# viniciusmenesessouza/VAE-GAN-based-model-for-image-generation-and-denoising

Hardware: AMD Instinct MI355X
Metric: images/sec/GPU VAE-GAN train step (higher is better)
Workload: dtype bf16; 1 GPU; CelebA-shaped 64x64 VAE-GAN full train step (E+G+5xD fwd, all bwd, 4 Adam), batch 128/GPU, global batch 128; img_size=64, per_gpu_batch=128, global_batch=128, parallelism=dp1, elide_dead_grads=False, hip_graph=True, hip_graph_segments=1

## Files before the change

vae-gan-based-model-for-image-generation-and-denoising_amd/csrc/bn_act.hip:

```cpp
#include "common.hpp"

namespace {

struct RedPlan { int nparts, rows_per_part, ncolblk; };

inline RedPlan plan_reduce(int64_t rows, int C) {
    const int cols = C / 4;
    const int ncol = cols < 256 ? cols : 256;
    const int rpp = 256 / ncol;
    const int64_t passes = (rows + rpp - 1) / rpp;
    int64_t np = passes / 8;
    if (np < 1) np = 1;
    if (np > 1024) np = 1024;
    int64_t rows_per_part = ((passes + np - 1) / np) * rpp;
    RedPlan p;
    p.nparts = (int)((rows + rows_per_part - 1) / rows_per_part);
    p.rows_per_part = (int)rows_per_part;
    p.ncolblk = (cols + 255) / 256;
    return p;
}

template <int DT, int MODE>
__global__ __launch_bounds__(256) void col_reduce_kernel(const void* __restrict__ x, const void* __restrict__ dy,
                                                         const float* __restrict__ scale,
// ... 169 lines not shown

__global__ __launch_bounds__(FIN_CH * FIN_PL) void bn_bwd_finalize_grouped_kernel(
    const float* __restrict__ partial, int nparts, int groups, int C, double count, const float* __restrict__ gamma,
    const float* __restrict__ coeffs, float* __restrict__ dgamma, float* __restrict__ dbeta, int accumulate,
    float* __restrict__ coef) {
    for (int g = 0; g < groups; ++g) {
        double s1, s2;
        int c;
        const bool lead = slab_sums(partial + (int64_t)g * nparts * 2 * C, nparts, C, s1, s2, c);
        if (lead) {
            const float fs1 = (float)s1, fs2 = (float)s2;
            const bool acc = accumulate || g > 0;
            if (dgamma) dgamma[c] = acc ? dgamma[c] + fs2 : fs2;
            if (dbeta) dbeta[c] = acc ? dbeta[c] + fs1 : fs1;
            const float a = (gamma ? gamma[c] : 1.f) * coeffs[(int64_t)g * 4 * C + C + c];
            float* cf = coef + (int64_t)g * 3 * C;
            cf[c] = a;
            cf[C + c] = (float)((double)a * s2 / count);
            cf[2 * C + c] = (float)((double)a * s1 / count);
        }
        __syncthreads();
    }
}

__global__ __launch_bounds__(FIN_CH * FIN_PL) void slab_sums_kernel(const float* __restrict__ slabs, int nparts, int C,
                                                                    double* __restrict__ sums) {
    double s1, s2;
    int c;
    if (!slab_sums(slabs, nparts, C, s1, s2, c)) return;
    sums[c] = s1;
    sums[C + c] = s2;
}

__global__ void bn_finalize_sums_kernel(const double* __restrict__ sums, int C, double count,
                                        const float* __restrict__ gamma, const float* __restrict__ beta,
                                        float* __restrict__ rmean, float* __restrict__ rvar, float momentum, float eps,
                                        float* __restrict__ mean, float* __restrict__ invstd,
                                        float* __restrict__ scale, float* __restrict__ shift) {
    const int c = blockIdx.x * blockDim.x + threadIdx.x;
    if (c >= C) return;
    const double mu = sums[c] / count;
    double var = sums[C + c] / count - mu * mu;
    if (var < 0.0) var = 0.0;
    const float is = (float)(1.0 / sqrt(var + (double)eps));
    const float muf = (float)mu;
    mean[c] = muf;
    invstd[c] = is;
    const float g = gamma ? gamma[c] : 1.f, b = beta ? beta[c] : 0.f;
    const float sc = g * is;
    scale[c] = sc;
    shift[c] = b - muf * sc;
    if (rmean) {
        const double unbiased = count > 1.0 ? var * (count / (count - 1.0)) : var;
        rmean[c] = (1.f - momentum) * rmean[c] + momentum * muf;
        rvar[c] = (1.f - momentum) * rvar[c] + momentum * (float)unbiased;
    }
}

__global__ void bn_bwd_finalize_sums_kernel(const double* __restrict__ gsums, const double* __restrict__ lsums, int C,
                                            double count, const float* __restrict__ gamma,
                                            const float* __restrict__ invstd, float* __restrict__ dgamma,
                                            float* __restrict__ dbeta, int accumulate, float* __restrict__ coef) {
    const int c = blockIdx.x * blockDim.x + threadIdx.x;
    if (c >= C) return;
    const float l1 = (float)lsums[c], l2 = (float)lsums[C + c];
    if (dgamma) dgamma[c] = accumulate ? dgamma[c] + l2 : l2;
    if (dbeta) dbeta[c] = accumulate ? dbeta[c] + l1 : l1;
    const float a = (gamma ? gamma[c] : 1.f) * invstd[c];
    coef[c] = a;
    coef[C + c] = (float)((double)a * gsums[C + c] / count);
    coef[2 * C + c] = (float)((double)a * gsums[c] / count);
}

__global__ void bn_eval_kernel(const float* gamma, const float* beta, const float* rmean, const float* rvar,
                               float eps, int C, float* scale, float* shift) {
    const int c = blockIdx.x * blockDim.x + threadIdx.x;
    if (c >= C) return;
    const float is = 1.f / sqrtf(rvar[c] + eps);
    const float sc = (gamma ? gamma[c] : 1.f) * is;
    scale[c] = sc;
    shift[c] = (beta ? beta[c] : 0.f) - rmean[c] * sc;
}

template <int DT>
__global__ __launch_bounds__(256) void bn_act_fwd_kernel(const void* __restrict__ x, void* __restrict__ y,
                                                         const float* __restrict__ scale,
                                                         const float* __restrict__ shift, int64_t nvec, int cols,
                                                         int act, float slope, int64_t nvec_per_group,
                                                         int64_t gstride, uint32_t* __restrict__ y8) {
    auto one = [&](int64_t i, float4 v) {
        const int c4 = (int)(i % cols) * 4;
        if (scale) {
            const int64_t go = (i / nvec_per_group) * gstride;
            const float4 sc = *reinterpret_cast<const float4*>(scale + go + c4);
            const float4 sh = *reinterpret_cast<const float4*>(shift + go + c4);
            v.x = sc.x * v.x + sh.x; v.y = sc.y * v.y + sh.y; v.z = sc.z * v.z + sh.z; v.w = sc.w * v.w + sh.w;
        }
        v.x = act_fwd(v.x, act, slope); v.y = act_fwd(v.y, act, slope);
        v.z = act_fwd(v.z, act, slope); v.w = act_fwd(v.w, act, slope);
        store4<DT>(y, i * 4, v);
        if (y8) {
            if constexpr (DT == VG_BF16) {
                v.x = ElemT<VG_BF16>::to_f32(ElemT<VG_BF16>::from_f32(v.x));
                v.y = ElemT<VG_BF16>::to_f32(ElemT<VG_BF16>::from_f32(v.y));
                v.z = ElemT<VG_BF16>::to_f32(ElemT<VG_BF16>::from_f32(v.z));
                v.w = ElemT<VG_BF16>::to_f32(ElemT<VG_BF16>::from_f32(v.w));
            }
            int w = __builtin_amdgcn_cvt_pk_fp8_f32(v.x, v.y, 0, false);
            w = __builtin_amdgcn_cvt_pk_fp8_f32(v.z, v.w, w, true);
            y8[i] = (uint32_t)w;
        }
    };
    const int64_t stride = (int64_t)gridDim.x * blockDim.x;
    int64_t i = (int64_t)blockIdx.x * blockDim.x + threadIdx.x;
    for (; i + 3 * stride < nvec; i += 4 * stride) {
        float4 v[4];
#pragma unroll
        for (int u = 0; u < 4; ++u) v[u] = load4<DT>(x, (i + u * stride) * 4);
#pragma unroll
        for (int u = 0; u < 4; ++u) one(i + u * stride, v[u]);
    }
    for (; i < nvec; i += stride) one(i, load4<DT>(x, i * 4));
}

__global__ __launch_bounds__(FIN_CH * FIN_PL) void bn_bwd_finalize_kernel(
    const float* __restrict__ partial, int nparts, int C, double count, const float* __restrict__ gamma,
    const float* __restrict__ invstd, float* __restrict__ dgamma, float* __restrict__ dbeta, int accumulate,
    float* __restrict__ coef) {
    double s1, s2;
    int c;
    if (!slab_sums(partial, nparts, C, s1, s2, c)) return;
    const float fs1 = (float)s1, fs2 = (float)s2;
    if (dgamma) dgamma[c] = accumulate ? dgamma[c] + fs2 : fs2;
    if (dbeta) dbeta[c] = accumulate ? dbeta[c] + fs1 : fs1;
    const float a = (gamma ? gamma[c] : 1.f) * invstd[c];
    coef[c] = a;
    coef[C + c] = (float)((double)a * s2 / count);
    coef[2 * C + c] = (float)((double)a * s1 / count);
}

template <int DT>
__global__ __launch_bounds__(256) void bn_act_bwd_apply_kernel(const void* __restrict__ x, const void* __restrict__ dy,
                                                               void* __restrict__ dx,
                                                               const float* __restrict__ scale,
                                                               const float* __restrict__ shift,
                                                               const float* __restrict__ mean,
                                                               const float* __restrict__ invstd,
                                                               const float* __restrict__ coef, int64_t nvec, int cols,
                                                               int C, int act, float slope, int64_t nvec_per_group,
                                                               int64_t gstride, int64_t cstride) {
    auto one = [&](int64_t i, const float4& v, const float4& g) {
        const int c4 = (int)(i % cols) * 4;
        const int64_t grp = i / nvec_per_group;
        const int64_t go = grp * gstride;
        const float* cf = coef + grp * cstride;
        const float4 sc = *reinterpret_cast<const float4*>(scale + go + c4);
        const float4 sh = *reinterpret_cast<const float4*>(shift + go + c4);
        const float4 mu = *reinterpret_cast<const float4*>(mean + go + c4);
        const float4 is = *reinterpret_cast<const float4*>(invstd + go + c4);
        const float4 ca = *reinterpret_cast<const float4*>(cf + c4);
        const float4 cbv = *reinterpret_cast<const float4*>(cf + C + c4);
        const float4 cc = *reinterpret_cast<const float4*>(cf + 2 * C + c4);
        float4 o;
        o.x = ca.x * act_bwd(sc.x * v.x + sh.x, g.x, act, slope) - cbv.x * ((v.x - mu.x) * is.x) - cc.x;
        o.y = ca.y * act_bwd(sc.y * v.y + sh.y, g.y, act, slope) - cbv.y * ((v.y - mu.y) * is.y) - cc.y;
        o.z = ca.z * act_bwd(sc.z * v.z + sh.z, g.z, act, slope) - cbv.z * ((v.z - mu.z) * is.z) - cc.z;
        o.w = ca.w * act_bwd(sc.w * v.w + sh.w, g.w, act, slope) - cbv.w * ((v.w - mu.w) * is.w) - cc.w;
        store4<DT>(dx, i * 4, o);
    };
    const int64_t stride = (int64_t)gridDim.x * blockDim.x;
    int64_t i = (int64_t)blockIdx.x * blockDim.x + threadIdx.x;
    for (; i + 3 * stride < nvec; i += 4 * stride) {
        float4 v[4], g[4];
#pragma unroll
        for (int u = 0; u < 4; ++u) { v[u] = load4<DT>(x, (i + u * stride) * 4); g[u] = load4<DT>(dy, (i + u * stride) * 4); }
#pragma unroll
        for (int u = 0; u < 4; ++u) one(i + u * stride, v[u], g[u]);
    }
    for (; i < nvec; i += stride) one(i, load4<DT>(x, i * 4), load4<DT>(dy, i * 4));
}

constexpr int FF_CH = 64, FF_PL = 16, FF_TH = FF_CH * FF_PL, FF_MAXPARTS = 200;
constexpr int64_t FF_MAXBYTES = 9ll << 20;

__device__ __forceinline__ void ff_slice_stats(const float* __restrict__ slabs, int nparts, int C, int c0, double count,
                                               double (*red)[FF_CH][2], double& mu_out, double& var_out) {
    const int ch = threadIdx.x & (FF_CH - 1), pl = threadIdx.x / FF_CH;
    double a = 0.0, b = 0.0;
    for (int p = pl; p < nparts; p += FF_PL) {
        a += (double)slabs[((int64_t)p * 2 + 0) * C + c0 + ch];
        b += (double)slabs[((int64_t)p * 2 + 1) * C + c0 + ch];
    }
    red[pl][ch][0] = a;
    red[pl][ch][1] = b;
    __syncthreads();
    double s1 = 0.0, s2 = 0.0;
#pragma unroll
    for (int k = 0; k < FF_PL; ++k) { s1 += red[k][ch][0]; s2 += red[k][ch][1]; }
    const double mu = s1 / count;
    double var = s2 / count - mu * mu;
    if (var < 0.0) var = 0.0;
    mu_out = mu;
    var_out = var;
    __syncthreads();
}

__global__ __launch_bounds__(FF_TH) void bn_fin_act_fwd_kernel(
    const uint16_t* __restrict__ x, uint16_t* __restrict__ y, const float* __restrict__ stats, int nparts, int groups,
    int C, double count, const float* __restrict__ gamma, const float* __restrict__ beta, float* __restrict__ rmean,
    float* __restrict__ rvar, float momentum, float eps, float* __restrict__ coeffs, int64_t rows_per_group,
    int rows_per_block, int act, float slope) {
    __shared__ double red[FF_PL][FF_CH][2];
    __shared__ float s_sc[FF_CH], s_sh[FF_CH];
    const int tid = threadIdx.x, ch = tid & (FF_CH - 1);
    const int c0 = blockIdx.y * FF_CH, grp = blockIdx.z;
    const bool lead = tid < FF_CH && c0 + ch < C;
    const float gm = (lead && gamma) ? gamma[c0 + ch] : 1.f, bt = (lead && beta) ? beta[c0 + ch] : 0.f;
    if (blockIdx.x == 0 && grp == 0) {
        float rm = (lead && rmean) ? rmean[c0 + ch] : 0.f, rv = (lead && rmean) ? rvar[c0 + ch] : 0.f;
        for (int g = 0; g < groups; ++g) {
            double mu, var;
            ff_slice_stats(stats + (int64_t)g * nparts * 2 * C, nparts, C, c0, count, red, mu, var);
            if (lead) {
                const float is = (float)(1.0 / sqrt(var + (double)eps));
                const float muf = (float)mu, sc = gm * is, sh = bt - muf * sc;
                float* co = coeffs + (int64_t)g * 4 * C + c0 + ch;
                co[0] = muf; co[C] = is; co[2 * C] = sc; co[3 * C] = sh;
                if (g == 0) { s_sc[ch] = sc; s_sh[ch] = sh; }
                if (rmean) {
                    const double unbiased = count > 1.0 ? var * (count / (count - 1.0)) : var;
                    rm = (1.f - momentum) * rm + momentum * muf;
                    rv = (1.f - momentum) * rv + momentum * (float)unbiased;
                }
            }
        }
        if (lead && rmean) { rmean[c0 + ch] = rm; rvar[c0 + ch] = rv; }
    } else {
        double mu, var;
        ff_slice_stats(stats + (int64_t)grp * nparts * 2 * C, nparts, C, c0, count, red, mu, var);
        if (lead) {
            const float is = (float)(1.0 / sqrt(var + (double)eps));
            const float muf = (float)mu, sc = gm * is;
            s_sc[ch] = sc;
            s_sh[ch] = bt - muf * sc;
        }
    }
    __syncthreads();
    const int u8 = (tid & 7) * 8, rl = tid >> 3;
    float sc[8], sh[8];
#pragma unroll
    for (int k = 0; k < 8; ++k) { sc[k] = s_sc[u8 + k]; sh[k] = s_sh[u8 + k]; }
    const int64_t r0 = (int64_t)blockIdx.x * rows_per_block;
    const int64_t r1 = r0 + rows_per_block < rows_per_group ? r0 + rows_per_block : rows_per_group;
    const int64_t base = (int64_t)grp * rows_per_group;
    if (c0 + u8 < C) {
        for (int64_t r = r0 + rl; r < r1; r += FF_TH / 8) {
            const int64_t off = (base + r) * C + c0 + u8;
            const u32x4 v = *reinterpret_cast<const u32x4*>(x + off);
            u32x4 o;
#pragma unroll
            for (int k2 = 0; k2 < 4; ++k2) {
                const float lo = act_fwd(sc[2 * k2] * __uint_as_float(v[k2] << 16) + sh[2 * k2], act, slope);
// ... 217 lines not shown
    return VG_LAUNCH_RC();
}

extern "C" int vg_bn_backward_finalize_sums(const double* global_sums, const double* local_sums, int C, int64_t count,
                                            const float* gamma, const float* invstd, float* dgamma, float* dbeta,
                                            int accumulate, float* coef, void* stream) {
    VG_CHECK_ARG(global_sums && local_sums && C > 0 && count > 0 && invstd && coef, VG_EINVAL);
    vg_launch_timed(4, bn_bwd_finalize_sums_kernel, dim3((C + 255) / 256), dim3(256), 0, vg_stream(stream),
                       global_sums, local_sums, C, (double)count, gamma, invstd, dgamma, dbeta, accumulate, coef);
    return VG_LAUNCH_RC();
}

extern "C" int vg_bn_eval_coeffs(const float* gamma, const float* beta, const float* running_mean,
                                 const float* running_var, float eps, int C, float* scale, float* shift,
                                 void* stream) {
    VG_CHECK_ARG(running_mean && running_var && scale && shift && C > 0, VG_EINVAL);
    vg_launch_timed(4, bn_eval_kernel, dim3((C + 63) / 64), dim3(64), 0, vg_stream(stream), gamma, beta, running_mean,
                       running_var, eps, C, scale, shift);
    return VG_LAUNCH_RC();
}

extern "C" int vg_bn_finalize_act_forward_supported(int nparts_per_group, int groups, int C, int64_t rows, int dtype) {
    return bn_fin_fwd_ok(nparts_per_group, groups, C, rows, dtype) ? 1 : 0;
}

extern "C" int vg_bn_finalize_act_forward(const void* x, void* y, const float* stats, int nparts_per_group, int groups,
                                          int C, int64_t rows, const float* gamma, const float* beta,
                                          float* running_mean, float* running_var, float momentum, float eps,
                                          float* coeffs, int act, float slope, int dtype, void* stream) {
    VG_CHECK_ARG(x && y && stats && coeffs && rows > 0 && C > 0, VG_EINVAL);
    VG_CHECK_ARG((running_mean == nullptr) == (running_var == nullptr), VG_EINVAL);
    VG_CHECK_ARG(vg_aligned16(x) && vg_aligned16(y), VG_EALIGN);
    if (!bn_fin_fwd_ok(nparts_per_group, groups, C, rows, dtype)) return VG_ENOSUP;
    const int64_t rpg = rows / groups;
    const int slices = C / FF_CH;
    int64_t want = 512 / (slices * groups);
    if (want < 1) want = 1;
    int64_t rpb = (rpg + want - 1) / want;
    rpb = (rpb + 127) / 128 * 128;
    const int rb = (int)((rpg + rpb - 1) / rpb);
    vg_launch_timed(4, bn_fin_act_fwd_kernel, dim3(rb, slices, groups), dim3(FF_TH), 0, vg_stream(stream),
                       reinterpret_cast<const uint16_t*>(x), reinterpret_cast<uint16_t*>(y), stats, nparts_per_group, groups,
                       C, (double)rpg, gamma, beta, running_mean, running_var, momentum, eps, coeffs, rpg, (int)rpb, act,
                       slope);
    return VG_LAUNCH_RC();
}

extern "C" int vg_bn_backward_finalize_apply(const void* x, const void* dy, void* dx, const float* partial,
                                             int nparts_per_group, int groups, int C, int64_t rows, const float* gamma,
                                             const float* coeffs, float* dgamma, float* dbeta, int accumulate, int act,
                                             float slope, int dtype, void* stream) {
    VG_CHECK_ARG(x && dy && dx && partial && coeffs && rows > 0 && C > 0, VG_EINVAL);
    VG_CHECK_ARG(vg_aligned16(x) && vg_aligned16(dy) && vg_aligned16(dx), VG_EALIGN);
    if (!bn_fin_fwd_ok(nparts_per_group, groups, C, rows, dtype)) return VG_ENOSUP;
    const int64_t rpg = rows / groups;
    const int slices = C / FF_CH;
    int64_t want = 512 / (slices * groups);
    if (want < 1) want = 1;
    int64_t rpb = (rpg + want - 1) / want;
    rpb = (rpb + 127) / 128 * 128;
    const int rb = (int)((rpg + rpb - 1) / rpb);
    vg_launch_timed(4, bn_bwd_fin_apply_kernel, dim3(rb, slices, groups), dim3(FF_TH), 0, vg_stream(stream),
                       reinterpret_cast<const uint16_t*>(x), reinterpret_cast<const uint16_t*>(dy),
                       reinterpret_cast<uint16_t*>(dx), partial, nparts_per_group, groups, C, (double)rpg, gamma, coeffs,
                       dgamma, dbeta, accumulate, rpg, (int)rpb, act, slope);
    return VG_LAUNCH_RC();
}

extern "C" int vg_bn_act_forward_fp8(const void* x, void* y, void* y8, const float* scale, const float* shift, int64_t rows,
                                     int C, int act, float slope, int groups, int64_t gstride, int dtype, void* stream);

extern "C" int vg_bn_act_forward(const void* x, void* y, const float* scale, const float* shift, int64_t rows, int C,
                                 int act, float slope, int groups, int64_t gstride, int dtype, void* stream) {
    return vg_bn_act_forward_fp8(x, y, nullptr, scale, shift, rows, C, act, slope, groups, gstride, dtype, stream);
}

extern "C" int vg_bn_act_forward_fp8(const void* x, void* y, void* y8, const float* scale, const float* shift, int64_t rows,
                                     int C, int act, float slope, int groups, int64_t gstride, int dtype, void* stream) {
    int rc = check_rows_c(x, rows, C, dtype);
    if (rc) return rc;
    VG_CHECK_ARG(y != nullptr && (scale == nullptr) == (shift == nullptr), VG_EINVAL);
    VG_CHECK_ARG(groups >= 1 && rows % groups == 0, VG_EINVAL);
    VG_CHECK_ARG(y8 == nullptr || (dtype == VG_BF16 && (reinterpret_cast<uintptr_t>(y8) & 3u) == 0), VG_EINVAL);
    const int64_t nvec = rows * C / 4;
    const int64_t nvg = nvec / groups;
    if (dtype == VG_F32)
        vg_launch_timed(4, bn_act_fwd_kernel<VG_F32>, dim3(ew_blocks(nvec)), dim3(256), 0, vg_stream(stream), x, y,
                           scale, shift, nvec, C / 4, act, slope, nvg, gstride, (uint32_t*)nullptr);
    else
        vg_launch_timed(4, bn_act_fwd_kernel<VG_BF16>, dim3(ew_blocks(nvec)), dim3(256), 0, vg_stream(stream), x, y,
                           scale, shift, nvec, C / 4, act, slope, nvg, gstride, reinterpret_cast<uint32_t*>(y8));
    return VG_LAUNCH_RC();
}

extern "C" int vg_channel_stats(const void* x, int64_t rows, int C, float* stats, int stats_capacity,
                                int* nparts_out, int dtype, void* stream) {
    int rc = check_rows_c(x, rows, C, dtype);
    if (rc) return rc;
    return launch_reduce<0>(x, nullptr, nullptr, nullptr, nullptr, nullptr, rows, C, 0, 0.f, stats, stats_capacity,
                            nparts_out, dtype, vg_stream(stream));
}

extern "C" int vg_bn_act_backward_reduce(const void* x, const void* dy, const float* scale, const float* shift,
                                         const float* mean, const float* invstd, int64_t rows, int C, int act,
                                         float slope, float* partial, int partial_capacity, int* nparts_out,
                                         int groups, int64_t gstride, int dtype, void* stream) {
    int rc = check_rows_c(x, rows, C, dtype);
    if (rc) return rc;
    VG_CHECK_ARG(dy && scale && shift && mean && invstd, VG_EINVAL);
    return launch_reduce<1>(x, dy, scale, shift, mean, invstd, rows, C, act, slope, partial, partial_capacity,
                            nparts_out, dtype, vg_stream(stream), groups, gstride);
}

extern "C" int vg_bn_backward_finalize(const float* partial, int nparts, int C, int64_t count, const float* gamma,
                                       const float* invstd, float* dgamma, float* dbeta, int accumulate, float* coef,
                                       void* stream) {
    VG_CHECK_ARG(partial && nparts > 0 && C > 0 && count > 0 && invstd && coef, VG_EINVAL);
    vg_launch_timed(4, bn_bwd_finalize_kernel, dim3((C + FIN_CH - 1) / FIN_CH), dim3(FIN_CH * FIN_PL), 0, vg_stream(stream), partial, nparts, C,
                       (double)count, gamma, invstd, dgamma, dbeta, accumulate, coef);
    return VG_LAUNCH_RC();
}

extern "C" int vg_bn_act_backward_apply(const void* x, const void* dy, void* dx, const float* scale,
                                        const float* shift, const float* mean, const float* invstd, const float* coef,
                                        int64_t rows, int C, int act, float slope, int groups, int64_t gstride,
                                        int64_t cstride, int dtype, void* stream) {
    int rc = check_rows_c(x, rows, C, dtype);
    if (rc) return rc;
    VG_CHECK_ARG(dy && dx && scale && shift && mean && invstd && coef, VG_EINVAL);
    VG_CHECK_ARG(groups >= 1 && rows % groups == 0, VG_EINVAL);
    const int64_t nvec = rows * C / 4;
    const int64_t nvg = nvec / groups;
    if (dtype == VG_F32)
        vg_launch_timed(4, bn_act_bwd_apply_kernel<VG_F32>, dim3(ew_blocks(nvec)), dim3(256), 0, vg_stream(stream), x,
                           dy, dx, scale, shift, mean, invstd, coef, nvec, C / 4, C, act, slope, nvg, gstride, cstride);
    else
        vg_launch_timed(4, bn_act_bwd_apply_kernel<VG_BF16>, dim3(ew_blocks(nvec)), dim3(256), 0, vg_stream(stream), x,
                           dy, dx, scale, shift, mean, invstd, coef, nvec, C / 4, C, act, slope, nvg, gstride, cstride);
    return VG_LAUNCH_RC();
}

extern "C" int vg_act_backward(const void* x, const void* dy, void* dx, int64_t n, int act, float slope, int dtype,
                               void* stream) {
    VG_CHECK_ARG(x && dy && dx && n > 0 && n % 4 == 0, VG_EINVAL);
    VG_CHECK_ARG(dtype == VG_F32 || dtype == VG_BF16, VG_ENOSUP);
    const int64_t nvec = n / 4;
    if (dtype == VG_F32)
        vg_launch_timed(4, act_bwd_kernel<VG_F32>, dim3(ew_blocks(nvec)), dim3(256), 0, vg_stream(stream), x, dy, dx,
                           nvec, act, slope);
    else
        vg_launch_timed(4, act_bwd_kernel<VG_BF16>, dim3(ew_blocks(nvec)), dim3(256), 0, vg_stream(stream), x, dy, dx,
                           nvec, act, slope);
    return VG_LAUNCH_RC();
}

extern "C" int vg_bias_grad(const void* dy, int64_t rows, int C, int NC, float* dbias, int accumulate, float* ws,
                            int ws_capacity, int dtype, void* stream) {
    int rc = check_rows_c(dy, rows, C, dtype);
    if (rc) return rc;
    VG_CHECK_ARG(dbias && ws && NC > 0 && NC <= C, VG_EINVAL);
    int nparts = 0;
    rc = launch_reduce<0>(dy, nullptr, nullptr, nullptr, nullptr, nullptr, rows, C, 0, 0.f, ws, ws_capacity, &nparts,
                          dtype, vg_stream(stream));
    if (rc) return rc;
    vg_launch_timed(4, bias_finalize_kernel, dim3((C + FIN_CH - 1) / FIN_CH), dim3(FIN_CH * FIN_PL), 0, vg_stream(stream), ws, nparts, C, NC,
                       dbias, accumulate);
    return VG_LAUNCH_RC();
}
```

vae-gan-based-model-for-image-generation-and-denoising_amd/csrc/common.hpp:

```cpp
#pragma once
#include <hip/hip_runtime.h>
#include <stdint.h>
#include "vaegan_hip.h"

typedef __attribute__((ext_vector_type(4))) float f32x4;
typedef __attribute__((ext_vector_type(8))) __bf16 bf16x8;
typedef __attribute__((ext_vector_type(4))) uint32_t u32x4;

#define VG_CHECK_ARG(cond, code) do { if (!(cond)) return (code); } while (0)

#include <atomic>
std::atomic<uint64_t>& vg_launch_counter();
#undef hipLaunchKernelGGL
#define hipLaunchKernelGGL(kernelName, numBlocks, numThreads, memPerBlock, streamId, ...)                       \
    do {                                                                                                        \
        vg_launch_counter().fetch_add(1, std::memory_order_relaxed);                                            \
        kernelName<<<(numBlocks), (numThreads), (memPerBlock), (streamId)>>>(__VA_ARGS__);                      \
    } while (0)
#define VG_LAUNCH_RC() ((int)hipGetLastError())

static inline hipStream_t vg_stream(void* s) { return reinterpret_cast<hipStream_t>(s); }
static inline bool vg_aligned16(const void* p) { return (reinterpret_cast<uintptr_t>(p) & 15u) == 0; }

template <int DT> struct ElemT;
// ... 50 lines not shown
}
template <int DT> __device__ __forceinline__ float load1(const void* base, int64_t idx) {
    return ElemT<DT>::to_f32(reinterpret_cast<const typename ElemT<DT>::type*>(base)[idx]);
}
template <int DT> __device__ __forceinline__ void store1(void* base, int64_t idx, float v) {
    reinterpret_cast<typename ElemT<DT>::type*>(base)[idx] = ElemT<DT>::from_f32(v);
}

__device__ __forceinline__ float act_fwd(float z, int act, float slope) {
    if (act == VG_ACT_RELU) return z > 0.f ? z : 0.f;
    if (act == VG_ACT_LRELU) return z > 0.f ? z : z * slope;
    return z;
}
__device__ __forceinline__ float act_bwd(float z, float g, int act, float slope) {
    if (act == VG_ACT_RELU) return z > 0.f ? g : 0.f;
    if (act == VG_ACT_LRELU) return z > 0.f ? g : g * slope;
    return g;
}

__device__ __forceinline__ float wave_sum(float v) {
#pragma unroll
    for (int o = 32; o > 0; o >>= 1) v += __shfl_xor(v, o);
    return v;
}
__device__ __forceinline__ double wave_sum_d(double v) {
#pragma unroll
    for (int o = 32; o > 0; o >>= 1) v += __shfl_xor(v, o);
    return v;
}

#include <hip/hip_ext.h>
#include <mutex>
#include <vector>
struct VgTiming {
    bool on = false;
    std::mutex mu;
    std::vector<hipEvent_t> pool;
    std::vector<std::pair<hipEvent_t, hipEvent_t>> rec[5];
};
VgTiming& vg_timing();

template <typename K, typename... Args>
inline void vg_launch_timed(int family, K kernel, dim3 grid, dim3 block, size_t shm, hipStream_t s, Args... args) {
    VgTiming& t = vg_timing();
    if (!t.on) {
        hipLaunchKernelGGL(kernel, grid, block, shm, s, args...);
        return;
    }
    hipEvent_t e0, e1;
    {
        std::lock_guard<std::mutex> g(t.mu);
        auto get = [&]() { hipEvent_t e; if (t.pool.empty()) { (void)hipEventCreate(&e); } else { e = t.pool.back(); t.pool.pop_back(); } return e; };
        e0 = get(); e1 = get();
        t.rec[family].push_back({e0, e1});
    }
    vg_launch_counter().fetch_add(1, std::memory_order_relaxed);
    hipExtLaunchKernelGGL(kernel, grid, block, shm, s, e0, e1, 0, args...);
}

struct VgSwitches {
    int gg_dma;
    int tile_min_wgs;
    int gg_patch;
    int gg_patch64;
    int gg_patch32;
    int gg_phase4;
    int gg_phase4_min;
    int gg_patch_nr3;
    int patch256_min;
    int patch256x64_min;
    int splitk_max_tiles;
    int splitk_general;
    int splitk_bigk;
    int splitk_wgs;
    int gg_nmajor;
    int edge;
    int wg_reduce_t;
    int wg_target;
    int wg_spec;
    int wg_dma;
    int wg_xcd;
    int bn_fused_fwd;
    int bn_onepass;
};
const VgSwitches& vg_sw();
```

vae-gan-based-model-for-image-generation-and-denoising_amd/csrc/pointwise.hip:

```cpp
#include "common.hpp"
#include "noise.hpp"

namespace {

__global__ __launch_bounds__(256) void cast_fp8_kernel(const u32x4* __restrict__ x, uint2* __restrict__ y, int64_t nvec,
                                                       float scale) {
    for (int64_t i = (int64_t)blockIdx.x * blockDim.x + threadIdx.x; i < nvec; i += (int64_t)gridDim.x * blockDim.x) {
        const u32x4 v = x[i];
        float f[8];
#pragma unroll
        for (int k = 0; k < 4; ++k) {
            f[2 * k] = __uint_as_float(v[k] << 16) * scale;
            f[2 * k + 1] = __uint_as_float(v[k] & 0xffff0000u) * scale;
        }
        uint2 o;
        int w = 0;
        w = __builtin_amdgcn_cvt_pk_fp8_f32(f[0], f[1], w, false);
        w = __builtin_amdgcn_cvt_pk_fp8_f32(f[2], f[3], w, true);
        o.x = (uint32_t)w;
        w = 0;
        w = __builtin_amdgcn_cvt_pk_fp8_f32(f[4], f[5], w, false);
        w = __builtin_amdgcn_cvt_pk_fp8_f32(f[6], f[7], w, true);
        o.y = (uint32_t)w;
        y[i] = o;
// ... 856 lines not shown
    VG_CHECK_ARG(B * groups <= HB_MAXROWS, VG_ENOSUP);
    DISPATCH_DT(head_bwd_kernel, dim3((K + 63) / 64), dim3(1024), vg_stream(stream), p, x, w, dx, dw, dlogit, B, groups,
                target0, target1, gscale, loss, accumulate_loss, accumulate_dw, K, C, HW);
    return VG_LAUNCH_RC();
}

extern "C" int vg_mean_forward_backward(const float* p, float sign, int B, float gscale, float* loss, int accumulate,
                                        float* dp, void* stream) {
    VG_CHECK_ARG(p && loss && B > 0, VG_EINVAL);
    hipLaunchKernelGGL(mean_loss_kernel, dim3(1), dim3(256), 0, vg_stream(stream), p, sign, B, gscale, loss, accumulate, dp);
    return VG_LAUNCH_RC();
}

extern "C" int vg_clamp(float* p, int64_t n, float lo, float hi, void* stream) {
    VG_CHECK_ARG(p && n > 0 && lo <= hi, VG_EINVAL);
    hipLaunchKernelGGL(clamp_kernel, dim3(blocks_for(n)), dim3(256), 0, vg_stream(stream), p, n, lo, hi);
    return VG_LAUNCH_RC();
}

extern "C" int vg_mse_forward_backward(const float* a, const float* b, int64_t n, float gscale, float* loss, float* d_a,
                                       float* ws, int ws_capacity, void* stream) {
    VG_CHECK_ARG(a && b && loss && ws && n > 0 && ws_capacity >= 1, VG_EINVAL);
    VG_CHECK_ARG(vg_aligned16(a) && vg_aligned16(b) && (d_a == nullptr || vg_aligned16(d_a)), VG_EALIGN);
    int blocks = blocks_for(n / 4, 1024);
    if (blocks > ws_capacity) blocks = ws_capacity;
    const float gcoef = (float)((double)gscale * 2.0 / (double)n);
    hipLaunchKernelGGL(mse_partial_kernel, dim3(blocks), dim3(256), 0, vg_stream(stream), a, b, n, gcoef, d_a, ws);
    int rc = VG_LAUNCH_RC();
    if (rc) return rc;
    hipLaunchKernelGGL(mse_final_kernel, dim3(1), dim3(64), 0, vg_stream(stream), ws, blocks, (double)n, loss);
    return VG_LAUNCH_RC();
}

extern "C" int vg_ssim(const float* a, const float* b, int B, int C, int H, int W, float* out, float* ws,
                       int ws_capacity, void* stream) {
    VG_CHECK_ARG(a && b && out && ws && B > 0 && C > 0 && H > 10 && W > 10 && ws_capacity >= 1, VG_EINVAL);
    const int64_t total = (int64_t)B * C * (H - 10) * (W - 10);
    int blocks = blocks_for(total, 1024);
    if (blocks > ws_capacity) blocks = ws_capacity;
    hipLaunchKernelGGL(ssim_kernel, dim3(blocks), dim3(256), 0, vg_stream(stream), a, b, B * C, H, W, ws);
    int rc = VG_LAUNCH_RC();
    if (rc) return rc;
    hipLaunchKernelGGL(mse_final_kernel, dim3(1), dim3(64), 0, vg_stream(stream), ws, blocks, (double)total, out);
    return VG_LAUNCH_RC();
}

extern "C" int vg_axpy(const float* a, const float* b, float alpha, float* out, int64_t n, void* stream) {
    VG_CHECK_ARG(a && b && out && n > 0, VG_EINVAL);
    hipLaunchKernelGGL(axpy_kernel, dim3(blocks_for(n)), dim3(256), 0, vg_stream(stream), a, b, alpha, out, n);
    return VG_LAUNCH_RC();
}

#include <cstdlib>
namespace {
VgSwitches g_sw;
int env_int(const char* name, int dflt) {
    const char* e = getenv(name);
    return e ? atoi(e) : dflt;
}
void read_switches() {
    g_sw.gg_dma = env_int("VG_GG_DMA", 1);
    g_sw.tile_min_wgs = env_int("VG_TILE_MIN_WGS", 512);
    g_sw.gg_patch = env_int("VG_GG_PATCH", 1);
    g_sw.gg_patch64 = env_int("VG_GG_PATCH64", 1);
    g_sw.gg_patch32 = env_int("VG_GG_PATCH32", 1);
    g_sw.gg_phase4 = env_int("VG_GG_PHASE4", 1);
    g_sw.gg_phase4_min = env_int("VG_GG_PHASE4_MIN", 512);
    g_sw.gg_patch_nr3 = env_int("VG_GG_PATCH_NR3", 1);
    g_sw.patch256_min = env_int("VG_PATCH256_MIN", 256);
    g_sw.patch256x64_min = env_int("VG_PATCH256X64_MIN", 512);
    g_sw.splitk_max_tiles = env_int("VG_SPLITK_MAX_TILES", 128);
    g_sw.splitk_wgs = env_int("VG_SPLITK_WGS", 1024);
    g_sw.splitk_bigk = env_int("VG_SPLITK_BIGK", 1);
    g_sw.splitk_general = env_int("VG_SPLITK_GENERAL", 0);
    g_sw.gg_nmajor = env_int("VG_GG_NMAJOR", 1);
    g_sw.edge = env_int("VG_EDGE", 1);
    g_sw.wg_reduce_t = env_int("VG_WG_REDUCE_T", 1);
    g_sw.wg_target = env_int("VG_WG_TARGET", 512);
    g_sw.wg_spec = env_int("VG_WG_SPEC", 3);
    g_sw.wg_dma = env_int("VG_WG_DMA", 1);
    g_sw.wg_xcd = env_int("VG_WG_XCD", 1);
    g_sw.bn_fused_fwd = env_int("VG_BN_FUSED_FWD", 1);
    g_sw.bn_onepass = env_int("VG_BN_ONEPASS", 0);
}
struct SwitchInit { SwitchInit() { read_switches(); } } g_switch_init;
}
const VgSwitches& vg_sw() { return g_sw; }
extern "C" int vg_reload_switches(void) {
    read_switches();
    return 0;
}

VgTiming& vg_timing() {
    static VgTiming t;
    return t;
}

std::atomic<uint64_t>& vg_launch_counter() {
    static std::atomic<uint64_t> n{0};
    return n;
}

extern "C" uint64_t vg_launch_count(void) { return vg_launch_counter().load(std::memory_order_relaxed); }

extern "C" int vg_timing_enable(int on) {
    VgTiming& t = vg_timing();
    std::lock_guard<std::mutex> g(t.mu);
    t.on = on != 0;
    return 0;
}

extern "C" int vg_timing_collect(int family, double* total_ms, int* launches) {
    VG_CHECK_ARG(family >= 0 && family < 5 && total_ms && launches, VG_EINVAL);
    VgTiming& t = vg_timing();
    std::lock_guard<std::mutex> g(t.mu);
    double sum = 0.0;
    for (auto& pr : t.rec[family]) {
        (void)hipEventSynchronize(pr.second);
        float ms = 0.f;
        if (hipEventElapsedTime(&ms, pr.first, pr.second) == hipSuccess) sum += ms;
        t.pool.push_back(pr.first);
        t.pool.push_back(pr.second);
    }
    *total_ms = sum;
    *launches = (int)t.rec[family].size();
    t.rec[family].clear();
    return 0;
}

extern "C" int vg_abi_version(void) { return VG_ABI_VERSION; }
extern "C" const char* vg_build_info(void) { return "vaegan_hip gfx950: gather-GEMM f32(16x16x4)/bf16(16x16x32) MFMA"; }
```

Baseline: 47980 images/sec.

## Restructure BN-activation apply kernels into row-blocked column-stationary streaming with wide vectors

```diff
diff --git a/vae-gan-based-model-for-image-generation-and-denoising_amd/csrc/bn_act.hip b/vae-gan-based-model-for-image-generation-and-denoising_amd/csrc/bn_act.hip
--- a/vae-gan-based-model-for-image-generation-and-denoising_amd/csrc/bn_act.hip
+++ b/vae-gan-based-model-for-image-generation-and-denoising_amd/csrc/bn_act.hip
@@ -275,45 +275,154 @@
     shift[c] = (beta ? beta[c] : 0.f) - rmean[c] * sc;
 }
 
-template <int DT>
+constexpr int EW_UNROLL = 4;
+constexpr int EW_FWD_WGS = 1024, EW_BWD_WGS = 768;
+inline bool stream_wide(int dtype, int64_t rows, int C) {
+    return dtype == VG_BF16 && C % 8 == 0 && rows * C * 2 >= (int64_t)vg_sw().bn_wide_min;
+}
+
+struct StreamPlan { int rows_per_block, blocks_per_group, ncolblk; };
+
+inline StreamPlan plan_stream(int64_t rows_per_group, int cols, int groups, int max_wgs) {
+    const int ncol = cols < 256 ? cols : 256;
+    const int rpp = 256 / ncol;
+    StreamPlan p;
+    p.ncolblk = (cols + 255) / 256;
+    const int64_t passes = (rows_per_group + rpp - 1) / rpp;
+    int64_t cap = max_wgs / ((int64_t)groups * p.ncolblk);
+    if (cap < 1) cap = 1;
+    const int64_t blocks = passes < cap ? passes : cap;
+    const int64_t rpb = (passes + blocks - 1) / blocks * rpp;
+    p.rows_per_block = (int)rpb;
+    p.blocks_per_group = (int)((rows_per_group + rpb - 1) / rpb);
+    return p;
+}
+
+template <int DT, int VW> struct RawVec { typedef __attribute__((ext_vector_type(VW / 2))) uint32_t type; };
+template <int VW> struct RawVec<VG_F32, VW> { typedef float4 type; };
+template <int DT, int VW>
+__device__ __forceinline__ typename RawVec<DT, VW>::type loadv(const void* base, int64_t idx) {
+    typedef typename RawVec<DT, VW>::type W;
+    return *reinterpret_cast<const W*>(reinterpret_cast<const typename ElemT<DT>::type*>(base) + idx);
+}
+template <int DT, int VW>
+__device__ __forceinline__ void unpackv(const typename RawVec<DT, VW>::type& r, float (&v)[VW]) {
+    if constexpr (DT == VG_F32) {
+        static_assert(VW == 4, "f32: one 16-byte vector");
+        v[0] = r.x; v[1] = r.y; v[2] = r.z; v[3] = r.w;
+    } else {
+#pragma unroll
+        for (int k = 0; k < VW / 2; ++k) {
+            v[2 * k] = __uint_as_float(r[k] << 16);
+            v[2 * k + 1] = __uint_as_float(r[k] & 0xffff0000u);
+        }
+    }
+}
+template <int DT, int VW> __device__ __forceinline__ void storev(void* base, int64_t idx, const float (&v)[VW]) {
+    typename RawVec<DT, VW>::type r;
+    if constexpr (DT == VG_F32) {
+        r = float4{v[0], v[1], v[2], v[3]};
+    } else {
+#pragma unroll
+        for (int k = 0; k < VW / 2; ++k)
+            r[k] = (uint32_t)ElemT<VG_BF16>::from_f32(v[2 * k]) | ((uint32_t)ElemT<VG_BF16>::from_f32(v[2 * k + 1]) << 16);
+    }
+    *reinterpret_cast<typename RawVec<DT, VW>::type*>(reinterpret_cast<typename ElemT<DT>::type*>(base) + idx) = r;
+}
+template <int V> struct IntC { static constexpr int value = V; };
+
+template <int VW> __device__ __forceinline__ void load_coef(const float* __restrict__ p, float (&c)[VW]) {
+#pragma unroll
+    for (int k = 0; k < VW; k += 4) {
+        const float4 r = *reinterpret_cast<const float4*>(p + k);
+        c[k] = r.x; c[k + 1] = r.y; c[k + 2] = r.z; c[k + 3] = r.w;
+    }
+}
+
+template <int VW>
+__device__ __forceinline__ void stream_range(int64_t rows, int C, int64_t rows_per_group, int rows_per_block, int& c,
+                                             int& rpp, int64_t& r0, int64_t& r1) {
+    const int cols = C / VW;
+    const int cb = blockIdx.y * 256;
+    const int ncol = min(256, cols - cb);
+    rpp = 256 / ncol;
+    const int tr = threadIdx.x / ncol, tc = threadIdx.x - tr * ncol;
+    c = (cb + tc) * VW;
+    const int64_t gbase = (int64_t)blockIdx.z * rows_per_group;
+    const int64_t b0 = gbase + (int64_t)blockIdx.x * rows_per_block;
+    r1 = min(min(rows, gbase + rows_per_group), b0 + (int64_t)rows_per_block);
+    r0 = tr < rpp ? b0 + tr : r1;
+}
+
+template <int DT, int VW>
 __global__ __launch_bounds__(256) void bn_act_fwd_kernel(const void* __restrict__ x, void* __restrict__ y,
                                                          const float* __restrict__ scale,
-                                                         const float* __restrict__ shift, int64_t nvec, int cols,
-                                                         int act, float slope, int64_t nvec_per_group,
-                                                         int64_t gstride, uint32_t* __restrict__ y8) {
-    auto one = [&](int64_t i, float4 v) {
-        const int c4 = (int)(i % cols) * 4;
-        if (scale) {
-            const int64_t go = (i / nvec_per_group) * gstride;
-            const float4 sc = *reinterpret_cast<const float4*>(scale + go + c4);
-            const float4 sh = *reinterpret_cast<const float4*>(shift + go + c4);
-            v.x = sc.x * v.x + sh.x; v.y = sc.y * v.y + sh.y; v.z = sc.z * v.z + sh.z; v.w = sc.w * v.w + sh.w;
-        }
-        v.x = act_fwd(v.x, act, slope); v.y = act_fwd(v.y, act, slope);
-        v.z = act_fwd(v.z, act, slope); v.w = act_fwd(v.w, act, slope);
-        store4<DT>(y, i * 4, v);
-        if (y8) {
-            if constexpr (DT == VG_BF16) {
-                v.x = ElemT<VG_BF16>::to_f32(ElemT<VG_BF16>::from_f32(v.x));
-                v.y = ElemT<VG_BF16>::to_f32(ElemT<VG_BF16>::from_f32(v.y));
-                v.z = ElemT<VG_BF16>::to_f32(ElemT<VG_BF16>::from_f32(v.z));
-                v.w = ElemT<VG_BF16>::to_f32(ElemT<VG_BF16>::from_f32(v.w));
-            }
-            int w = __builtin_amdgcn_cvt_pk_fp8_f32(v.x, v.y, 0, false);
-            w = __builtin_amdgcn_cvt_pk_fp8_f32(v.z, v.w, w, true);
-            y8[i] = (uint32_t)w;
+                                                         const float* __restrict__ shift, int64_t rows, int C, int act,
+                                                         float slope, int64_t rows_per_group, int rows_per_block,
+                                                         int64_t gstride, uint8_t* __restrict__ y8) {
+    int c, rpp;
+    int64_t r, r1;
+    stream_range<VW>(rows, C, rows_per_group, rows_per_block, c, rpp, r, r1);
+    typedef typename RawVec<DT, VW>::type Raw;
+    const int64_t step = (int64_t)rpp * C;
+    int64_t off = r * C + c;
+    float sc[VW], sh[VW];
+    if (scale) {
+        load_coef<VW>(scale + (int64_t)blockIdx.z * gstride + c, sc);
+        load_coef<VW>(shift + (int64_t)blockIdx.z * gstride + c, sh);
+    }
+    auto run = [&](auto act_c, auto affine_c) {
+        constexpr int ACT = decltype(act_c)::value;
+        constexpr bool AFFINE = decltype(affine_c)::value;
+        auto one = [&](int64_t o, const Raw& raw) {
+            float f[VW];
+            unpackv<DT, VW>(raw, f);
+            if (AFFINE) {
+#pragma unroll
+                for (int k = 0; k < VW; ++k) f[k] = __builtin_fmaf(sc[k], f[k], sh[k]);
+            }
+#pragma unroll
+            for (int k = 0; k < VW; ++k) f[k] = act_fwd(f[k], ACT, slope);
+            storev<DT, VW>(y, o, f);
+            if (y8) {
+                if constexpr (DT == VG_BF16) {
+#pragma unroll
+                    for (int k = 0; k < VW; ++k) f[k] = ElemT<VG_BF16>::to_f32(ElemT<VG_BF16>::from_f32(f[k]));
+                }
+                typedef __attribute__((ext_vector_type(VW / 4))) uint32_t W8;
+                W8 w8;
+#pragma unroll
+                for (int k = 0; k < VW / 4; ++k) {
+                    int w = __builtin_amdgcn_cvt_pk_fp8_f32(f[4 * k], f[4 * k + 1], 0, false);
+                    w = __builtin_amdgcn_cvt_pk_fp8_f32(f[4 * k + 2], f[4 * k + 3], w, true);
+                    w8[k] = (uint32_t)w;
+                }
+                *reinterpret_cast<W8*>(y8 + o) = w8;
+            }
+        };
+        for (; r + (EW_UNROLL - 1) * rpp < r1; r += EW_UNROLL * rpp, off += EW_UNROLL * step) {
+            Raw v[EW_UNROLL];
+#pragma unroll
+            for (int u = 0; u < EW_UNROLL; ++u) v[u] = loadv<DT, VW>(x, off + u * step);
+#pragma unroll
+            for (int u = 0; u < EW_UNROLL; ++u) one(off + u * step, v[u]);
+        }
+        if (r < r1) {
+            Raw v[EW_UNROLL - 1];
+#pragma unroll
+            for (int u = 0; u < EW_UNROLL - 1; ++u)
+                if (r + u * rpp < r1) v[u] = loadv<DT, VW>(x, off + u * step);
+#pragma unroll
+            for (int u = 0; u < EW_UNROLL - 1; ++u)
+                if (r + u * rpp < r1) one(off + u * step, v[u]);
         }
     };
-    const int64_t stride = (int64_t)gridDim.x * blockDim.x;
-    int64_t i = (int64_t)blockIdx.x * blockDim.x + threadIdx.x;
-    for (; i + 3 * stride < nvec; i += 4 * stride) {
-        float4 v[4];
-#pragma unroll
-        for (int u = 0; u < 4; ++u) v[u] = load4<DT>(x, (i + u * stride) * 4);
-#pragma unroll
-        for (int u = 0; u < 4; ++u) one(i + u * stride, v[u]);
-    }
-    for (; i < nvec; i += stride) one(i, load4<DT>(x, i * 4));
+    auto with_act = [&](auto affine_c) {
+        if (act == VG_ACT_RELU) run(IntC<VG_ACT_RELU>{}, affine_c);
+        else if (act == VG_ACT_LRELU) run(IntC<VG_ACT_LRELU>{}, affine_c);
+        else run(IntC<VG_ACT_NONE>{}, affine_c);
+    };
+    if (scale) with_act(IntC<1>{}); else with_act(IntC<0>{});
 }
 
 __global__ __launch_bounds__(FIN_CH * FIN_PL) void bn_bwd_finalize_kernel(
@@ -332,45 +441,66 @@
     coef[2 * C + c] = (float)((double)a * s1 / count);
 }
 
-template <int DT>
+template <int DT, int VW>
 __global__ __launch_bounds__(256) void bn_act_bwd_apply_kernel(const void* __restrict__ x, const void* __restrict__ dy,
                                                                void* __restrict__ dx,
                                                                const float* __restrict__ scale,
                                                                const float* __restrict__ shift,
                                                                const float* __restrict__ mean,
                                                                const float* __restrict__ invstd,
-                                                               const float* __restrict__ coef, int64_t nvec, int cols,
-                                                               int C, int act, float slope, int64_t nvec_per_group,
-                                                               int64_t gstride, int64_t cstride) {
-    auto one = [&](int64_t i, const float4& v, const float4& g) {
-        const int c4 = (int)(i % cols) * 4;
-        const int64_t grp = i / nvec_per_group;
-        const int64_t go = grp * gstride;
-        const float* cf = coef + grp * cstride;
-        const float4 sc = *reinterpret_cast<const float4*>(scale + go + c4);
-        const float4 sh = *reinterpret_cast<const float4*>(shift + go + c4);
-        const float4 mu = *reinterpret_cast<const float4*>(mean + go + c4);
-        const float4 is = *reinterpret_cast<const float4*>(invstd + go + c4);
-        const float4 ca = *reinterpret_cast<const float4*>(cf + c4);
-        const float4 cbv = *reinterpret_cast<const float4*>(cf + C + c4);
-        const float4 cc = *reinterpret_cast<const float4*>(cf + 2 * C + c4);
-        float4 o;
-        o.x = ca.x * act_bwd(sc.x * v.x + sh.x, g.x, act, slope) - cbv.x * ((v.x - mu.x) * is.x) - cc.x;
-        o.y = ca.y * act_bwd(sc.y * v.y + sh.y, g.y, act, slope) - cbv.y * ((v.y - mu.y) * is.y) - cc.y;
-        o.z = ca.z * act_bwd(sc.z * v.z + sh.z, g.z, act, slope) - cbv.z * ((v.z - mu.z) * is.z) - cc.z;
-        o.w = ca.w * act_bwd(sc.w * v.w + sh.w, g.w, act, slope) - cbv.w * ((v.w - mu.w) * is.w) - cc.w;
-        store4<DT>(dx, i * 4, o);
+                                                               const float* __restrict__ coef, int64_t rows, int C,
+                                                               int act, float slope, int64_t rows_per_group,
+                                                               int rows_per_block, int64_t gstride, int64_t cstride) {
+    int c, rpp;
+    int64_t r, r1;
+    stream_range<VW>(rows, C, rows_per_group, rows_per_block, c, rpp, r, r1);
+    typedef typename RawVec<DT, VW>::type Raw;
+    const int64_t step = (int64_t)rpp * C;
+    int64_t off = r * C + c;
+    float sc[VW], sh[VW], mu[VW], is[VW], ca[VW], cbv[VW], cc[VW];
+    const int64_t go = (int64_t)blockIdx.z * gstride + c;
+    const float* cf = coef + (int64_t)blockIdx.z * cstride + c;
+    load_coef<VW>(scale + go, sc);
+    load_coef<VW>(shift + go, sh);
+    load_coef<VW>(mean + go, mu);
+    load_coef<VW>(invstd + go, is);
+    load_coef<VW>(cf, ca);
+    load_coef<VW>(cf + C, cbv);
+    load_coef<VW>(cf + 2 * C, cc);
+    auto run = [&](auto act_c) {
+        constexpr int ACT = decltype(act_c)::value;
+        auto one = [&](int64_t o, const Raw& rx, const Raw& rg) {
+            float f[VW], d[VW], q[VW];
+            unpackv<DT, VW>(rx, f);
+            unpackv<DT, VW>(rg, d);
+#pragma unroll
+            for (int k = 0; k < VW; ++k) {
+                const float dz = act_bwd(__builtin_fmaf(sc[k], f[k], sh[k]), d[k], ACT, slope);
+                const float xh = cbv[k] * ((f[k] - mu[k]) * is[k]);
+                q[k] = __builtin_fmaf(ca[k], dz, -xh) - cc[k];
+            }
+            storev<DT, VW>(dx, o, q);
+        };
+        for (; r + (EW_UNROLL - 1) * rpp < r1; r += EW_UNROLL * rpp, off += EW_UNROLL * step) {
+            Raw v[EW_UNROLL], g[EW_UNROLL];
+#pragma unroll
+            for (int u = 0; u < EW_UNROLL; ++u) { v[u] = loadv<DT, VW>(x, off + u * step); g[u] = loadv<DT, VW>(dy, off + u * step); }
+#pragma unroll
+            for (int u = 0; u < EW_UNROLL; ++u) one(off + u * step, v[u], g[u]);
+        }
+        if (r < r1) {
+            Raw v[EW_UNROLL - 1], g[EW_UNROLL - 1];
+#pragma unroll
+            for (int u = 0; u < EW_UNROLL - 1; ++u)
+                if (r + u * rpp < r1) { v[u] = loadv<DT, VW>(x, off + u * step); g[u] = loadv<DT, VW>(dy, off + u * step); }
+#pragma unroll
+            for (int u = 0; u < EW_UNROLL - 1; ++u)
+                if (r + u * rpp < r1) one(off + u * step, v[u], g[u]);
+        }
     };
-    const int64_t stride = (int64_t)gridDim.x * blockDim.x;
-    int64_t i = (int64_t)blockIdx.x * blockDim.x + threadIdx.x;
-    for (; i + 3 * stride < nvec; i += 4 * stride) {
-        float4 v[4], g[4];
-#pragma unroll
-        for (int u = 0; u < 4; ++u) { v[u] = load4<DT>(x, (i + u * stride) * 4); g[u] = load4<DT>(dy, (i + u * stride) * 4); }
-#pragma unroll
-        for (int u = 0; u < 4; ++u) one(i + u * stride, v[u], g[u]);
-    }
-    for (; i < nvec; i += stride) one(i, load4<DT>(x, i * 4), load4<DT>(dy, i * 4));
+    if (act == VG_ACT_RELU) run(IntC<VG_ACT_RELU>{});
+    else if (act == VG_ACT_LRELU) run(IntC<VG_ACT_LRELU>{});
+    else run(IntC<VG_ACT_NONE>{});
 }
 
 constexpr int FF_CH = 64, FF_PL = 16, FF_TH = FF_CH * FF_PL, FF_MAXPARTS = 200;
@@ -754,14 +884,22 @@
     VG_CHECK_ARG(y != nullptr && (scale == nullptr) == (shift == nullptr), VG_EINVAL);
     VG_CHECK_ARG(groups >= 1 && rows % groups == 0, VG_EINVAL);
     VG_CHECK_ARG(y8 == nullptr || (dtype == VG_BF16 && (reinterpret_cast<uintptr_t>(y8) & 3u) == 0), VG_EINVAL);
-    const int64_t nvec = rows * C / 4;
-    const int64_t nvg = nvec / groups;
+    const int64_t rpg = rows / groups;
+    const hipStream_t s = vg_stream(stream);
+    uint8_t* twin = reinterpret_cast<uint8_t*>(y8);
+    const bool wide = stream_wide(dtype, rows, C) && vg_aligned16(x) &&
+                      vg_aligned16(y) && (reinterpret_cast<uintptr_t>(y8) & 7u) == 0;
+    const StreamPlan p = plan_stream(rpg, C / (wide ? 8 : 4), groups, EW_FWD_WGS);
+    const dim3 grid(p.blocks_per_group, p.ncolblk, groups);
     if (dtype == VG_F32)
-        vg_launch_timed(4, bn_act_fwd_kernel<VG_F32>, dim3(ew_blocks(nvec)), dim3(256), 0, vg_stream(stream), x, y,
-                           scale, shift, nvec, C / 4, act, slope, nvg, gstride, (uint32_t*)nullptr);
+        vg_launch_timed(4, (bn_act_fwd_kernel<VG_F32, 4>), grid, dim3(256), 0, s, x, y, scale, shift, rows, C, act, slope,
+                           rpg, p.rows_per_block, gstride, twin);
+    else if (wide)
+        vg_launch_timed(4, (bn_act_fwd_kernel<VG_BF16, 8>), grid, dim3(256), 0, s, x, y, scale, shift, rows, C, act, slope,
+                           rpg, p.rows_per_block, gstride, twin);
     else
-        vg_launch_timed(4, bn_act_fwd_kernel<VG_BF16>, dim3(ew_blocks(nvec)), dim3(256), 0, vg_stream(stream), x, y,
-                           scale, shift, nvec, C / 4, act, slope, nvg, gstride, reinterpret_cast<uint32_t*>(y8));
+        vg_launch_timed(4, (bn_act_fwd_kernel<VG_BF16, 4>), grid, dim3(256), 0, s, x, y, scale, shift, rows, C, act, slope,
+                           rpg, p.rows_per_block, gstride, twin);
     return VG_LAUNCH_RC();
 }
 
@@ -801,14 +939,21 @@
     if (rc) return rc;
     VG_CHECK_ARG(dy && dx && scale && shift && mean && invstd && coef, VG_EINVAL);
     VG_CHECK_ARG(groups >= 1 && rows % groups == 0, VG_EINVAL);
-    const int64_t nvec = rows * C / 4;
-    const int64_t nvg = nvec / groups;
+    const int64_t rpg = rows / groups;
+    const hipStream_t s = vg_stream(stream);
+    const bool wide = stream_wide(dtype, rows, C) && vg_aligned16(x) &&
+                      vg_aligned16(dy) && vg_aligned16(dx);
+    const StreamPlan p = plan_stream(rpg, C / (wide ? 8 : 4), groups, EW_BWD_WGS);
+    const dim3 grid(p.blocks_per_group, p.ncolblk, groups);
     if (dtype == VG_F32)
-        vg_launch_timed(4, bn_act_bwd_apply_kernel<VG_F32>, dim3(ew_blocks(nvec)), dim3(256), 0, vg_stream(stream), x,
-                           dy, dx, scale, shift, mean, invstd, coef, nvec, C / 4, C, act, slope, nvg, gstride, cstride);
+        vg_launch_timed(4, (bn_act_bwd_apply_kernel<VG_F32, 4>), grid, dim3(256), 0, s, x, dy, dx, scale, shift, mean, invstd,
+                           coef, rows, C, act, slope, rpg, p.rows_per_block, gstride, cstride);
+    else if (wide)
+        vg_launch_timed(4, (bn_act_bwd_apply_kernel<VG_BF16, 8>), grid, dim3(256), 0, s, x, dy, dx, scale, shift, mean, invstd,
+                           coef, rows, C, act, slope, rpg, p.rows_per_block, gstride, cstride);
     else
-        vg_launch_timed(4, bn_act_bwd_apply_kernel<VG_BF16>, dim3(ew_blocks(nvec)), dim3(256), 0, vg_stream(stream), x,
-                           dy, dx, scale, shift, mean, invstd, coef, nvec, C / 4, C, act, slope, nvg, gstride, cstride);
+        vg_launch_timed(4, (bn_act_bwd_apply_kernel<VG_BF16, 4>), grid, dim3(256), 0, s, x, dy, dx, scale, shift, mean, invstd,
+                           coef, rows, C, act, slope, rpg, p.rows_per_block, gstride, cstride);
     return VG_LAUNCH_RC();
 }
 
diff --git a/vae-gan-based-model-for-image-generation-and-denoising_amd/csrc/common.hpp b/vae-gan-based-model-for-image-generation-and-denoising_amd/csrc/common.hpp
--- a/vae-gan-based-model-for-image-generation-and-denoising_amd/csrc/common.hpp
+++ b/vae-gan-based-model-for-image-generation-and-denoising_amd/csrc/common.hpp
@@ -156,5 +156,6 @@
     int wg_xcd;
     int bn_fused_fwd;
     int bn_onepass;
+    int bn_wide_min;
 };
 const VgSwitches& vg_sw();
diff --git a/vae-gan-based-model-for-image-generation-and-denoising_amd/csrc/pointwise.hip b/vae-gan-based-model-for-image-generation-and-denoising_amd/csrc/pointwise.hip
--- a/vae-gan-based-model-for-image-generation-and-denoising_amd/csrc/pointwise.hip
+++ b/vae-gan-based-model-for-image-generation-and-denoising_amd/csrc/pointwise.hip
@@ -962,6 +962,7 @@
     g_sw.wg_xcd = env_int("VG_WG_XCD", 1);
     g_sw.bn_fused_fwd = env_int("VG_BN_FUSED_FWD", 1);
     g_sw.bn_onepass = env_int("VG_BN_ONEPASS", 0);
+    g_sw.bn_wide_min = env_int("VG_BN_WIDE_MIN", 4 << 20);
 }
 struct SwitchInit { SwitchInit() { read_switches(); } } g_switch_init;
 }
```

Measured after the change: 49090 images/sec (median of 6 runs). +2.3%, better.
